# nanoporetech/tombo

Hardware: NVIDIA H100
Metric: resquiggle_reads_per_sec (higher is better)
Workload: dtype f64

## Files before the change

### tombo_b200/csrc/dp_row.cuh

```cuda
#pragma once
#include "common.cuh"

struct DpConsts {
    double z_shift, stay_pen, skip_pen, mhz;
    int winsor;
};

struct RowSpec {
    const double *em;
    const double *zrow;
    double mu, sd;
    tb2_rcp inv_sd;
    int e0;
    int lo, hi;
    double maskval;
};

__device__ __forceinline__ double tb2_zscore(const RowSpec &rs, const DpConsts &c, int j)
{
    if (rs.zrow) return rs.zrow[j];
    if (j < rs.lo || j >= rs.hi) return rs.maskval;
    double a = tb2_div_by(fabs(__ldg(rs.em + (rs.e0 + j)) - rs.mu), rs.sd, rs.inv_sd);
    if (c.winsor) a = (c.mhz < a) ? c.mhz : a;
    return c.z_shift - a;
}

template <int WPL, bool FIX>
__device__ __forceinline__ void tb2_walk(const double *prev, double *cur, int W, int chunk,
                                         int lane, int nvalid, const RowSpec &rs,
                                         const DpConsts &c, int d, bool first_skip, double x,
                                         uint32_t (&codes)[WPL], double &best, int &best_idx,
                                         double &x_end)
{
    const int j0 = lane * chunk;
    int p = j0 + d;
    int lane_p = p / chunk;
    int i_p = p - lane_p * chunk;
    double pm1 = tb2_neg_inf();
    if (p >= 1 && p - 1 < W) {
        const int q = p - 1, lq = q / chunk;
        pm1 = prev[(q - lq * chunk) * 32 + lq];
    }
    bool done = false;
#pragma unroll
    for (int w = 0; w < WPL; ++w) {
        const int ibeg = w * 16;
        const int iend = min(nvalid, ibeg + 16);
        uint32_t cw = FIX ? codes[w] : 0u;
        for (int i = ibeg; i < iend && !done; ++i) {
            const int j = j0 + i;
            const double z = tb2_zscore(rs, c, j);
            const double pv = (p < W) ? prev[i_p * 32 + lane_p] : tb2_neg_inf();
            double nx;
            uint32_t code;
            if (j == 0) {
                if (first_skip) { nx = pv - c.skip_pen; code = 1u; }
                else { nx = pm1 + z; code = 2u; }
            } else {
                const double a = (x - c.stay_pen) + z;
                double cc = pm1 + z;
                uint32_t cf = 2u;
                const double sk = pv - c.skip_pen;
                if (sk > cc) { cc = sk; cf = 1u; }
                if (cc > a) { nx = cc; code = cf; }
                else { nx = a; code = 0u; }
            }
            const int sh = 2 * (i - ibeg);
            if (FIX) {
                const double old = cur[i * 32 + lane];
                cw = (cw & ~(3u << sh)) | (code << sh);
                if (nx == old) done = true;
            } else {
                cw |= code << sh;
            }
            cur[i * 32 + lane] = nx;
            if (nx > best || (FIX && nx == best && j < best_idx)) { best = nx; best_idx = j; }
            x = nx;
            pm1 = pv;
            ++p;
            if (++i_p == chunk) { i_p = 0; ++lane_p; }
        }
        codes[w] = cw;
    }
    if (!done && nvalid > 0) x_end = x;
}

template <int WPL>
__device__ __forceinline__ void tb2_dp_row(const double *prev, double *cur, int W, int chunk,
                                           int lane, const RowSpec &rs, const DpConsts &c,
                                           int d, bool first_skip, uint32_t (&codes)[WPL],
                                           double &best, int &best_idx)
{
    const int nvalid = max(0, min(chunk, W - lane * chunk));
    best = tb2_neg_inf();
    best_idx = 0x7fffffff;
    double x_end = tb2_neg_inf();
    tb2_walk<WPL, false>(prev, cur, W, chunk, lane, nvalid, rs, c, d, first_skip, tb2_neg_inf(),
                         codes, best, best_idx, x_end);
    double last_in = tb2_neg_inf();
    for (;;) {
        const double xin = __shfl_up_sync(TB2_FULL_MASK, x_end, 1);
        const bool need = (lane > 0) && (nvalid > 0) && (xin != last_in);
        if (!__any_sync(TB2_FULL_MASK, need)) break;
        if (need) {
            tb2_walk<WPL, true>(prev, cur, W, chunk, lane, nvalid, rs, c, d, first_skip, xin,
                                codes, best, best_idx, x_end);
            last_in = xin;
        }
    }
}

__device__ __forceinline__ int tb2_warp_argmax(double best, int best_idx)
{
#pragma unroll
    for (int off = 16; off > 0; off >>= 1) {
        const double ob = __shfl_xor_sync(TB2_FULL_MASK, best, off);
        const int oi = __shfl_xor_sync(TB2_FULL_MASK, best_idx, off);
        if (ob > best || (ob == best && oi < best_idx)) { best = ob; best_idx = oi; }
    }
    return best_idx;
}

__device__ unsigned long long g_tb2_dp_counters[8];

#ifdef TB2_EMUL
__device__ __forceinline__ double tb2_lds(unsigned a) { return *(double *)emul_shared_ptr(a); }
__device__ __forceinline__ void tb2_sts(unsigned a, double v) { *(double *)emul_shared_ptr(a) = v; }
#else
__device__ __forceinline__ double tb2_lds(unsigned a)
{
    double v;
    asm volatile("ld.shared.f64 %0, [%1];" : "=d"(v) : "r"(a));
    return v;
}
__device__ __forceinline__ void tb2_sts(unsigned a, double v)
{
    asm volatile("st.shared.f64 [%0], %1;" ::"r"(a), "d"(v));
}
#endif

__device__ __forceinline__ void tb2_dp_row_s(unsigned prev_s, unsigned cur_s, unsigned z_s,
                                             unsigned c_s, int W, int chunk, int lane,
                                             const RowSpec &rs, const DpConsts &c, int d,
                                             bool first_skip, uint32_t &codeword, double &best,
                                             int &best_idx)
{
    const double NEG = tb2_neg_inf();
    const double stay = c.stay_pen, skip = c.skip_pen;
    const int j0 = lane * chunk;
    const int nvalid = max(0, min(chunk, W - j0));
    const unsigned lo8 = 8u * (unsigned)lane;
    cur_s += lo8; z_s += lo8; c_s += lo8;
    uint32_t cfw = 0u, cw = 0u;
    int p = j0 + d;
    int lane_p = p / chunk;
    int i_p = p - lane_p * chunk;
    double pm1 = NEG;
    if (p >= 1 && p - 1 < W) {
        const int q = p - 1, lq = q / chunk;
        pm1 = tb2_lds(prev_s + 8u * (unsigned)((q - lq * chunk) * 32 + lq));
    }
    double x = NEG;
    best = NEG;
    best_idx = 0x7fffffff;
#pragma unroll 1
    for (int i = 0; i < nvalid; ++i) {
        const int j = j0 + i;
        const double zz = tb2_zscore(rs, c, j);
        const double pv = (p < W) ? tb2_lds(prev_s + 8u * (unsigned)(i_p * 32 + lane_p)) : NEG;
        double cand = pm1 + zz;
        uint32_t cf = 2u;
        const double sk = pv - skip;
        double a;
        if (j == 0) {
            a = NEG;
            if (first_skip) { cand = sk; cf = 1u; }
        } else {
            if (sk > cand) { cand = sk; cf = 1u; }
            a = (x - stay) + zz;
        }
        double nx = a;
        uint32_t code = 0u;
        if (cand > a) { nx = cand; code = cf; }
        const unsigned off = 256u * (unsigned)i;
        tb2_sts(z_s + off, zz);
        tb2_sts(c_s + off, cand);
        tb2_sts(cur_s + off, nx);
        cfw |= cf << (2 * i);
        cw |= code << (2 * i);
        if (nx > best) { best = nx; best_idx = j; }
        x = nx;
        pm1 = pv;
        ++p;
        if (++i_p == chunk) { i_p = 0; ++lane_p; }
    }
    double x_end = x;
    double last_in = NEG;
    int n_rounds = 0, n_walked = 0;
    for (;;) {
        const double xin = __shfl_up_sync(TB2_FULL_MASK, x_end, 1);
        const bool need = (lane > 0) && (nvalid > 0) && (xin != last_in);
        if (!__any_sync(TB2_FULL_MASK, need)) break;
        ++n_rounds;
        if (need) {
            double xx = xin;
            bool done = false;
#pragma unroll 1
            for (int i = 0; i < nvalid; ++i) {
                ++n_walked;
                const unsigned off = 256u * (unsigned)i;
                const double a = (xx - stay) + tb2_lds(z_s + off);
                const double cand = tb2_lds(c_s + off);
                double nx = a;
                uint32_t code = 0u;
                if (cand > a) { nx = cand; code = (cfw >> (2 * i)) & 3u; }
                const double old = tb2_lds(cur_s + off);
                cw = (cw & ~(3u << (2 * i))) | (code << (2 * i));
                const int j = j0 + i;
                if (nx > best || (nx == best && j < best_idx)) { best = nx; best_idx = j; }
                xx = nx;
                if (nx == old) { done = true; break; }
                tb2_sts(cur_s + off, nx);
            }
            if (!done) x_end = xx;
            last_in = xin;
        }
    }
    codeword = cw;
#ifdef TB2_DP_COUNTERS
    n_walked = __reduce_add_sync(TB2_FULL_MASK, n_walked);
    if (lane == 0) {
        atomicAdd(&g_tb2_dp_counters[0], 1ULL);
        atomicAdd(&g_tb2_dp_counters[1], (unsigned long long)n_rounds);
        atomicAdd(&g_tb2_dp_counters[2], (unsigned long long)n_walked);
        if (n_rounds > 2) atomicAdd(&g_tb2_dp_counters[3], 1ULL);
    }
#else
    (void)n_rounds; (void)n_walked;
#endif
}

enum { TB2_MODE_PLAIN = 0, TB2_MODE_MASKED = 1, TB2_MODE_ADAPTIVE = 2, TB2_MODE_EXPLICIT = 3 };

struct PassCtx {
    int W, chunk;
    double *buf0, *buf1;
    double *zbuf, *cbuf;
    const double *em;
    int n_em;
    const double *rm, *rs_;
    const double *zmat;
    int mso;
    double msp_start, msp_stop;
    double mask_shifted;
    double mask_fill;
    int *starts;
    uint32_t *tb;
    double *ring;
    double *dbg_fwd;
    long long *dbg_tb;
};

#define TB2_MASK_BASES 50

template <int WPL>
__device__ __noinline__ int tb2_run_rows(const PassCtx &pc, const DpConsts &c, int mode, int r_begin,
                            int r_end, int n_bases_total, int *cur_sel, int *argmax_out)
{
    const int lane = tb2_lane();
    const int W = pc.W, chunk = pc.chunk;
    double *prev = (*cur_sel) ? pc.buf1 : pc.buf0;
    double *cur = (*cur_sel) ? pc.buf0 : pc.buf1;
    int last_argmax = *argmax_out;
    const bool fast_s = (pc.zbuf != nullptr) && __isShared(pc.buf0);
    const unsigned z_s = fast_s ? (unsigned)__cvta_generic_to_shared(pc.zbuf) : 0u;
    const unsigned c_s = fast_s ? (unsigned)__cvta_generic_to_shared(pc.cbuf) : 0u;
    int prev_start = (r_begin > 0) ? pc.starts[r_begin - 1] : 0;
    const int half_bw = W / 2;
    for (int r = r_begin; r < r_end; ++r) {
        RowSpec rs;
        rs.em = pc.em; rs.zrow = nullptr;
        rs.mu = pc.rm ? __ldg(pc.rm + r) : 0.0;
        rs.sd = pc.rs_ ? __ldg(pc.rs_ + r) : 1.0;
        rs.inv_sd = tb2_rcp_of(rs.sd);
        rs.lo = 0; rs.hi = W; rs.maskval = pc.mask_fill;
        int cur_start;
        if (mode == TB2_MODE_ADAPTIVE) {
            cur_start = prev_start + last_argmax - half_bw + 1;
            if (cur_start < prev_start) cur_start = prev_start;
            if (cur_start >= pc.n_em) {
                if (r < n_bases_total - 2) return TB2_ERR_ADAPTIVE_BEYOND_SIGNAL;
                cur_start = pc.n_em - 1;
            }
            if (lane == 0) pc.starts[r] = cur_start;
            rs.hi = min(W, pc.n_em - cur_start);
        } else {
            cur_start = pc.starts[r];
            if (mode == TB2_MODE_MASKED) {
                const int sml = max(pc.mso - cur_start, 0);
                int eml = 0;
                if (r < TB2_MASK_BASES) {
                    const int msp = (int)tb2_linspace_at(pc.msp_start, pc.msp_stop,
                                                         TB2_MASK_BASES, r);
                    eml = W - (msp - cur_start);
                }
                if (cur_start + W - eml > pc.n_em) eml = cur_start + W - pc.n_em;
                rs.lo = sml; rs.hi = W - eml; rs.maskval = pc.mask_shifted;
            } else if (mode == TB2_MODE_EXPLICIT) {
                rs.zrow = pc.zmat + (size_t)r * W;
            }
        }
        rs.e0 = cur_start;
        const int d = (r > 0) ? cur_start - prev_start : 0;
        const bool first_skip = (r == 0) || (d == 0);
        uint32_t codes[WPL];
        double best; int best_idx;
        if (WPL == 1 && fast_s)
            tb2_dp_row_s((unsigned)__cvta_generic_to_shared(prev), (unsigned)__cvta_generic_to_shared(cur),
                         z_s, c_s, W, chunk, lane, rs, c, d, first_skip, codes[0], best, best_idx);
        else
            tb2_dp_row<WPL>(prev, cur, W, chunk, lane, rs, c, d, first_skip, codes, best, best_idx);
#pragma unroll
        for (int w = 0; w < WPL; ++w)
            pc.tb[(size_t)r * (WPL * 32) + w * 32 + lane] = codes[w];
        if (mode == TB2_MODE_ADAPTIVE || r == r_end - 1 || r == n_bases_total - 1)
            last_argmax = tb2_warp_argmax(best, best_idx);
        __syncwarp();
        if (pc.dbg_fwd) {
            const int nvalid = max(0, min(chunk, W - lane * chunk));
            for (int i = 0; i < nvalid; ++i) {
                const int j = lane * chunk + i;
                pc.dbg_fwd[(size_t)(r + 1) * W + j] = cur[i * 32 + lane];
                uint32_t cwv = codes[0];
#pragma unroll
                for (int k = 1; k < WPL; ++k) if ((i >> 4) == k) cwv = codes[k];
                pc.dbg_tb[(size_t)(r + 1) * W + j] = (cwv >> (2 * (i & 15))) & 3u;
            }
        }
        double *t = prev; prev = cur; cur = t;
        *cur_sel ^= 1;
        prev_start = cur_start;
    }
    *argmax_out = last_argmax;
    return TB2_OK;
}

__device__ __forceinline__ void tb2_init_row0(const PassCtx &pc, int *cur_sel)
{
    const int lane = tb2_lane();
    for (int i = 0; i < pc.chunk; ++i) pc.buf0[i * 32 + lane] = 0.0;
    *cur_sel = 0;
    __syncwarp();
}

__device__ __forceinline__ void tb2_load_row(const PassCtx &pc, const double *row, int *cur_sel)
{
    const int lane = tb2_lane();
    for (int j = lane; j < pc.W; j += 32) {
        const int lj = j / pc.chunk;
        pc.buf0[(j - lj * pc.chunk) * 32 + lj] = row[j];
    }
    *cur_sel = 0;
    __syncwarp();
}

template <int WPL>
__device__ __forceinline__ uint32_t tb2_tb_code(const uint32_t (&w)[WPL], int bp, int chunk)
{
    const int lj = bp / chunk;
    const int i = bp - lj * chunk;
    uint32_t v = w[0];
#pragma unroll
    for (int k = 1; k < WPL; ++k) if ((i >> 4) == k) v = w[k];
    v = __shfl_sync(TB2_FULL_MASK, v, lj);
    return (v >> (2 * (i & 15))) & 3u;
}

template <int WPL>
__device__ __noinline__ int tb2_tb_seg_chunk(const uint32_t *tb, const int *starts, int row_hi, int row_lo,
                                int W, int chunk, int thresh, int *cur_event_io, int *read_tb)
{
    const int lane = tb2_lane();
    int cur_event = *cur_event_io;
    int sp = row_hi;
    while (sp > row_lo) {
        const int nblk = min(4, sp - row_lo);
        uint32_t w[4][WPL];
        int st[4];
#pragma unroll
        for (int b = 0; b < 4; ++b) {
            if (b < nblk) {
                const int row = sp - 1 - b;
#pragma unroll
                for (int k = 0; k < WPL; ++k)
                    w[b][k] = tb[(size_t)row * (WPL * 32) + k * 32 + lane];
                st[b] = starts[row];
            }
        }
#pragma unroll
        for (int b = 0; b < 4; ++b) {
            if (b < nblk) {
                int bp = cur_event - st[b];
                if (bp < 0 || bp >= W) return TB2_ERR_UNEXPECTED;
                uint32_t code = tb2_tb_code<WPL>(w[b], bp, chunk);
                while (code == 0u) {
                    --bp;
                    if (bp < 0) return TB2_ERR_UNEXPECTED;
                    code = tb2_tb_code<WPL>(w[b], bp, chunk);
                }
                if (code == 2u) --bp;
                if (thresh >= 0 && min(bp, W - bp - 1) < thresh)
                    return TB2_ERR_BEYOND_BANDWIDTH;
                cur_event = st[b] + bp;
                if (lane == 0) read_tb[sp - 1 - b] = cur_event + 1;
            }
        }
        sp -= nblk;
    }
    *cur_event_io = cur_event;
    __syncwarp();
    return TB2_OK;
}

__device__ __forceinline__ int tb2_wf_strip_words(const int *starts, int s0, int r_end, int W)
{
    const int last = min(31, r_end - 1 - s0);
    const int span = starts[s0 + last] - starts[s0] + W - 1 + last;
    return span < 0 ? -1 : ((span >> 4) + 1) * 32;
}

__device__ long long tb2_wf_total_words(const int *starts, int r_end, int W)
{
    long long sum = 0;
    int bad = 0;
    for (int s0 = tb2_lane() * 32; s0 < r_end; s0 += 32 * 32) {
        const int w = tb2_wf_strip_words(starts, s0, r_end, W);
        if (w < 0) bad = 1; else sum += w;
    }
#pragma unroll
    for (int off = 16; off > 0; off >>= 1) sum += __shfl_xor_sync(TB2_FULL_MASK, sum, off);
    return __any_sync(TB2_FULL_MASK, bad) ? -1 : sum;
}

template <int MODE, bool WIN>
__device__ __forceinline__ double tb2_wf_z(const double *ep, int j, double mu, double sd,
                                           tb2_rcp inv_sd, int lo, int hi, double maskval,
                                           const double *zrow, double zs, double mhz)
{
    if (MODE == TB2_MODE_EXPLICIT) return zrow[j];
    if (MODE == TB2_MODE_MASKED && (j < lo || j >= hi)) return maskval;
    double a = tb2_div_by(fabs(__ldg(ep) - mu), sd, inv_sd);
    if (WIN) a = (mhz < a) ? mhz : a;
    return zs - a;
}

template <bool RBS>
__device__ __forceinline__ double tb2_rb_ld(const double *rb, unsigned rb_s, int i)
{
    if (RBS) return tb2_lds(rb_s + 8u * (unsigned)i);
    return rb[i];
}
template <bool RBS>
__device__ __forceinline__ void tb2_rb_st(double *rb, unsigned rb_s, int i, double v)
{
    if (RBS) tb2_sts(rb_s + 8u * (unsigned)i, v);
    else rb[i] = v;
}

#define TB2_WF_MOVE_BITS(code, q) ((((code) != 0u ? 1u : 0u) << (q)) | (((code) == 1u ? 0x10000u : 0u) << (q)))

#ifdef TB2_EMUL
#define TB2_WF_PLD(up, U) if (l0flag) up = tb2_lds(rd_a + 8 * (U));
#else
#define TB2_WF_PLD(up, U)                                                                       \
        asm volatile("{ .reg .pred p; setp.ne.u32 p, %2, 0; @p ld.shared.f64 %0, [%1+%3]; }"    \
                     : "+d"(up) : "r"(rd_a), "r"(l0flag), "n"(8 * (U)));
#endif
#define TB2_WF_FAST_STEP(U)                                                                     \
    {                                                                                           \
        double up;                                                                              \
        if ((U) == 0) {                                                                         \
            up = __shfl_up_sync(TB2_FULL_MASK, xout, 1);                                        \
            TB2_WF_PLD(up, U)                                                                   \
        } else up = tb2_lds(rd_a + 8u * (U));                                                   \
        __syncwarp();                                                                           \
        const double zn = tb2_wf_z<MODE, WIN>(ep + (U) + 1, j + (U) + 1, mu, sd, inv_sd, lo,    \
                                              hi, maskval, nullptr, zs, mhz);                   \
        const double a = (x - stay) + z;                                                        \
        double cc = up_prev + z;                                                                \
        const double sk = up - skip;                                                            \
        if (sk > cc) { cc = sk; cw |= 0x10000u << (U); }                                        \
        double nx = a;                                                                          \
        if (cc > a) { nx = cc; cw |= 1u << (U); }                                               \
        up_prev = up;                                                                           \
        x = nx; xout = nx; z = zn;                                                              \
        tb2_sts(wr_a + 8u * (U), nx);                                                           \
        __syncwarp();                                                                           \
    }

template <int MODE, bool DBG, bool WIN, bool RBS>
__device__ __noinline__ int tb2_wavefront_rows_t(const PassCtx &pc, const DpConsts &c, int r_end,
                                                 double *rowbuf, uint32_t *tbw, int *argmax_out)
{
    const int lane = tb2_lane();
    const int W = pc.W;
    const double NEG = tb2_neg_inf();
    const double stay = c.stay_pen, skip = c.skip_pen, zs = c.z_shift, mhz = c.mhz;
    const unsigned rb_s = RBS ? (unsigned)__cvta_generic_to_shared(rowbuf) : 0u;
    const unsigned ring_s = (RBS && pc.ring) ? (unsigned)__cvta_generic_to_shared(pc.ring) : 0u;
    const double *em = pc.em;
    const int *starts = pc.starts;
    constexpr bool FAST_T = RBS && !DBG && MODE != TB2_MODE_EXPLICIT;
    const bool FAST = FAST_T && pc.ring != nullptr;
    if (FAST) {
        for (int jj = lane; jj < W; jj += 32) tb2_rb_st<RBS>(rowbuf, rb_s, jj, 0.0);
        __syncwarp();
    }
    uint32_t *tbs = tbw;
    for (int s0 = 0; s0 < r_end; s0 += 32) {
        const int r = s0 + lane;
        const bool row_ok = r < r_end;
        const int lane_last = min(31, r_end - 1 - s0);
        const int rr = min(r, r_end - 1);
        const int start = starts[rr];
        const int prev_start = rr > 0 ? starts[rr - 1] : start;
        const int d = start - prev_start;
        const double mu = pc.rm ? __ldg(pc.rm + rr) : 0.0;
        const double sd = pc.rs_ ? __ldg(pc.rs_ + rr) : 1.0;
        const tb2_rcp inv_sd = tb2_rcp_of(sd);
        int lo = 0, hi = W;
        double maskval = pc.mask_fill;
        if (MODE == TB2_MODE_MASKED && row_ok) {
            const int sml = max(pc.mso - start, 0);
            int eml = 0;
            if (r < TB2_MASK_BASES)
                eml = W - ((int)tb2_linspace_at(pc.msp_start, pc.msp_stop, TB2_MASK_BASES, r) - start);
            if (start + W - eml > pc.n_em) eml = start + W - pc.n_em;
            lo = sml; hi = W - eml; maskval = pc.mask_shifted;
        }
        const double *zrow = (MODE == TB2_MODE_EXPLICIT && row_ok) ? pc.zmat + (size_t)r * W : nullptr;
        const bool first_skip = (r == 0) || (d == 0);
        const bool is_tail = row_ok && (lane == lane_last);
        const int start_first = __shfl_sync(TB2_FULL_MASK, start, 0);
        const int start_last = __shfl_sync(TB2_FULL_MASK, start, lane_last);
        int dmax = row_ok ? d : 0, dmin = row_ok ? d : 0;
#pragma unroll
        for (int off = 16; off > 0; off >>= 1) {
            dmax = max(dmax, __shfl_xor_sync(TB2_FULL_MASK, dmax, off));
            dmin = min(dmin, __shfl_xor_sync(TB2_FULL_MASK, dmin, off));
        }
        const bool lean = FAST && dmin >= 0;
        const int t_begin = start_first;
        const int t_end = start_last + W - 1 + lane_last;
        int t_lo = start_last + lane_last + 1, t_hi = start_first + W - 2 - dmax;
        if (!lean) { t_lo = t_end + 1; t_hi = t_end; }
        double x = 0.0, xout = 0.0, up_prev = 0.0;
        uint32_t cw = 0u;
        const int lane_eff = min(lane, lane_last);
        int j = t_begin - lane_eff - start;
        const double *ep = em + (t_begin - lane_eff);
        int t = t_begin;
        const int w_act = row_ok ? W : 0;
        const int julo = d >= 1 ? 1 : 0, jllo = 1 - julo;
        const unsigned n_u = (unsigned)max(W - d - julo, 0), n_ul = (unsigned)max(W - d - jllo + 1, 0);
#define TB2_WF_LEAN_STEP()                                                                      \
        {                                                                                       \
            double up = __shfl_up_sync(TB2_FULL_MASK, xout, 1);                                 \
            if (lane == 0 && (unsigned)(j + d) < (unsigned)W) up = tb2_rb_ld<RBS>(rowbuf, rb_s, j + d); \
            const double upl = up_prev;                                                         \
            up_prev = up;                                                                       \
            const bool act = (unsigned)j < (unsigned)w_act;                                     \
            const double u = ((unsigned)(j - julo) < n_u) ? up : NEG;                           \
            const double ul = ((unsigned)(j - jllo) < n_ul) ? upl : NEG;                        \
            const double z = act ? tb2_wf_z<MODE, WIN>(ep, j, mu, sd, inv_sd, lo, hi, maskval,  \
                                                       zrow, zs, mhz) : 0.0;                    \
            const double a = (x - stay) + z;                                                    \
            double cc = ul + z;                                                                 \
            uint32_t code = 2u;                                                                 \
            const double sk = u - skip;                                                         \
            if (sk > cc) { cc = sk; code = 1u; }                                                \
            double nx = a;                                                                      \
            if (cc > a) nx = cc; else code = 0u;                                                \
            const int tq = (t - t_begin) & 15;                                                  \
            if (act) {                                                                          \
                x = nx; xout = nx;                                                              \
                cw |= TB2_WF_MOVE_BITS(code, tq);                                               \
                if (is_tail) tb2_rb_st<RBS>(rowbuf, rb_s, j, nx);                               \
            }                                                                                   \
            if (tq == 15 || t == t_end) {                                                       \
                tbs[((t - t_begin) >> 4) * 32 + lane] = cw;                                     \
                cw = 0u;                                                                        \
            }                                                                                   \
              \
              \
            __syncwarp();                                                                       \
            ++j; ++ep;                                                                          \
        }
        if (lean) {
            x = NEG;
            if (lane == 0 && d >= 1) up_prev = tb2_rb_ld<RBS>(rowbuf, rb_s, d - 1);
            for (; t <= t_end && (t < t_lo || ((t - t_begin) & 15) != 0); ++t) TB2_WF_LEAN_STEP()
        }
#define TB2_WF_GENERAL_STEP()                                                                   \
        {                                                                                       \
            double up = __shfl_up_sync(TB2_FULL_MASK, xout, 1);                                 \
            const int p = j + d;                                                                \
            double upl = up_prev;                                                               \
            if (lane == 0) {                                                                    \
                if (s0 == 0) { up = 0.0; upl = 0.0; }                                           \
                else {                                                                          \
                    up = (p >= 0 && p < W) ? tb2_rb_ld<RBS>(rowbuf, rb_s, p) : NEG;             \
                    if (j == 0) upl = (p >= 1 && p - 1 < W) ? tb2_rb_ld<RBS>(rowbuf, rb_s, p - 1) : NEG; \
                }                                                                               \
            }                                                                                   \
            up_prev = up;                                                                       \
            const int tq = (t - t_begin) & 15;                                                  \
            if (row_ok && j >= 0 && j < W) {                                                    \
                const double z = tb2_wf_z<MODE, WIN>(ep, j, mu, sd, inv_sd, lo, hi, maskval,    \
                                                     zrow, zs, mhz);                            \
                const double u = (p < W) ? up : NEG;                                            \
                const double ul = (p >= 1 && p - 1 < W) ? upl : NEG;                            \
                double nx;                                                                      \
                uint32_t code;                                                                  \
                if (j == 0) {                                                                   \
                    if (first_skip) { nx = u - skip; code = 1u; }                               \
                    else { nx = ul + z; code = 2u; }                                            \
                } else {                                                                        \
                    const double a = (x - stay) + z;                                            \
                    double cc = ul + z;                                                         \
                    uint32_t cf = 2u;                                                           \
                    const double sk = u - skip;                                                 \
                    if (sk > cc) { cc = sk; cf = 1u; }                                          \
                    if (cc > a) { nx = cc; code = cf; }                                         \
                    else { nx = a; code = 0u; }                                                 \
                }                                                                               \
                x = nx;                                                                         \
                xout = nx;                                                                      \
                cw |= TB2_WF_MOVE_BITS(code, tq);                                               \
                if (is_tail) tb2_rb_st<RBS>(rowbuf, rb_s, j, nx);                               \
                if (DBG) {                                                                      \
                    pc.dbg_fwd[(size_t)(r + 1) * W + j] = nx;                                   \
                    pc.dbg_tb[(size_t)(r + 1) * W + j] = code;                                  \
                }                                                                               \
            }                                                                                   \
            if (!DBG && (tq == 15 || t == t_end)) {                                             \
                tbs[((t - t_begin) >> 4) * 32 + lane] = cw;                                     \
                cw = 0u;                                                                        \
            }                                                                                   \
            __syncwarp();                                                                       \
            ++j; ++ep;                                                                          \
        }
        if (lean && t + 15 <= t_hi) {
            double z = tb2_wf_z<MODE, WIN>(ep, j, mu, sd, inv_sd, lo, hi, maskval, nullptr, zs, mhz);
            unsigned rd_a = lane == 0 ? rb_s + 8u * (unsigned)(j + d) : ring_s + 8u * (unsigned)(lane - 2);
            unsigned wr_a = is_tail ? rb_s + 8u * (unsigned)j : ring_s + 8u * (unsigned)lane;
            const unsigned rd_inc = lane == 0 ? 128u : 0u, wr_inc = is_tail ? 128u : 0u;
            const unsigned l0flag = lane == 0;
            uint32_t *tbp = tbs + ((t - t_begin) >> 4) * 32 + lane;
            for (; t + 15 <= t_hi; t += 16) {
                TB2_WF_FAST_STEP(0) TB2_WF_FAST_STEP(1) TB2_WF_FAST_STEP(2) TB2_WF_FAST_STEP(3)
                TB2_WF_FAST_STEP(4) TB2_WF_FAST_STEP(5) TB2_WF_FAST_STEP(6) TB2_WF_FAST_STEP(7)
                TB2_WF_FAST_STEP(8) TB2_WF_FAST_STEP(9) TB2_WF_FAST_STEP(10) TB2_WF_FAST_STEP(11)
                TB2_WF_FAST_STEP(12) TB2_WF_FAST_STEP(13) TB2_WF_FAST_STEP(14) TB2_WF_FAST_STEP(15)
                *tbp = cw;
                cw = 0u;
                tbp += 32;
                rd_a += rd_inc; wr_a += wr_inc;
                j += 16; ep += 16;
            }
            cw = 0u;
        }
        if (lean) {
            for (; t <= t_end; ++t) TB2_WF_LEAN_STEP()
        } else {
            for (; t <= t_end; ++t) TB2_WF_GENERAL_STEP()
        }
#undef TB2_WF_GENERAL_STEP
#undef TB2_WF_LEAN_STEP
        tbs += (((t_end - t_begin) >> 4) + 1) * 32;
        __syncwarp();
    }
    double best = NEG;
    int best_idx = 0x7fffffff;
    for (int jj = lane; jj < W; jj += 32) {
        const double v = tb2_rb_ld<RBS>(rowbuf, rb_s, jj);
        if (v > best) { best = v; best_idx = jj; }
    }
    *argmax_out = tb2_warp_argmax(best, best_idx);
    return TB2_OK;
}
#undef TB2_WF_FAST_STEP

__device__ int tb2_wavefront_rows(const PassCtx &pc, const DpConsts &c, int mode, int r_end,
                                  double *rowbuf, uint32_t *tbw, int *argmax_out)
{
    const bool rbs = __isShared(rowbuf);
    const bool win = c.winsor != 0;
#define TB2_WF_CALL(M, D, WN, RB) tb2_wavefront_rows_t<M, D, WN, RB>(pc, c, r_end, rowbuf, tbw, argmax_out)
    if (mode == TB2_MODE_EXPLICIT) {
        if (pc.dbg_fwd) return rbs ? TB2_WF_CALL(TB2_MODE_EXPLICIT, true, false, true)
                                   : TB2_WF_CALL(TB2_MODE_EXPLICIT, true, false, false);
        return TB2_ERR_INVALID_ARG;
    }
    if (mode == TB2_MODE_MASKED) {
        if (win) return rbs ? TB2_WF_CALL(TB2_MODE_MASKED, false, true, true)
                            : TB2_WF_CALL(TB2_MODE_MASKED, false, true, false);
        return rbs ? TB2_WF_CALL(TB2_MODE_MASKED, false, false, true)
                   : TB2_WF_CALL(TB2_MODE_MASKED, false, false, false);
    }
    if (win) return rbs ? TB2_WF_CALL(TB2_MODE_PLAIN, false, true, true)
                        : TB2_WF_CALL(TB2_MODE_PLAIN, false, true, false);
    return rbs ? TB2_WF_CALL(TB2_MODE_PLAIN, false, false, true)
               : TB2_WF_CALL(TB2_MODE_PLAIN, false, false, false);
#undef TB2_WF_CALL
}

__device__ __noinline__ int tb2_tb_seg_wf(const uint32_t *tbw, long long total_words, const int *starts,
                             int n_rows, int W, int thresh, int *cur_event_io, int *read_tb)
{
    const int lane = tb2_lane();
    int cur_event = *cur_event_io;
    const uint32_t *tbs = tbw + total_words;
    for (int s0 = ((n_rows - 1) >> 5) << 5; s0 >= 0; s0 -= 32) {
        const int nblk = min(32, n_rows - s0);
        const int sw = tb2_wf_strip_words(starts, s0, n_rows, W);
        if (sw < 0) return TB2_ERR_UNEXPECTED;
        tbs -= sw;
        const int nw = sw >> 5;
        const int t_begin = starts[s0];
        const float slope = (float)(cur_event - starts[0]) / (float)(s0 + nblk);
        int my_start = 0, base = 0;
        uint32_t w0 = 0, w1 = 0, w2 = 0;
        if (lane < nblk) {
            my_start = starts[s0 + lane];
            const int est = cur_event - (int)((float)(nblk - 1 - lane) * slope) + lane - t_begin;
            base = min(max((est >> 4) - 1, 0), max(nw - 3, 0));
            const uint32_t *rw = tbs + lane;
            w0 = rw[base * 32];
            if (base + 1 < nw) w1 = rw[(base + 1) * 32];
            if (base + 2 < nw) w2 = rw[(base + 2) * 32];
        }
        for (int k = nblk - 1; k >= 0; --k) {
            const int row = s0 + k;
            const int st = __shfl_sync(TB2_FULL_MASK, my_start, k);
            const int bs = __shfl_sync(TB2_FULL_MASK, base, k);
            int bp = cur_event - st;
            if (bp < 0 || bp >= W) return TB2_ERR_UNEXPECTED;
            const int toff = st + k - t_begin;
            uint32_t code;
            for (;;) {
                const int ts = bp + toff;
                const int wi = ts >> 4, rel = wi - bs, q = ts & 15;
                uint32_t v;
                if (rel >= 0 && rel < 3) {
                    const uint32_t mine = rel == 0 ? w0 : (rel == 1 ? w1 : w2);
                    v = __shfl_sync(TB2_FULL_MASK, mine, k);
                } else {
                    v = tbs[wi * 32 + k];
                }
                const uint32_t nz = (v & 0xffffu) & (0xffffu >> (15 - q));
                if (nz != 0u) {
                    const int kq = 31 - __clz(nz);
                    bp -= q - kq;
                    code = ((v >> (16 + kq)) & 1u) ? 1u : 2u;
                    break;
                }
                bp -= q + 1;
                if (bp < 0) return TB2_ERR_UNEXPECTED;
            }
            if (code == 2u) --bp;
            if (thresh >= 0 && min(bp, W - bp - 1) < thresh) return TB2_ERR_BEYOND_BANDWIDTH;
            cur_event = st + bp;
            if (lane == 0) read_tb[row] = cur_event + 1;
        }
    }
    *cur_event_io = cur_event;
    __syncwarp();
    return TB2_OK;
}
```

Measured before the change: 686,500.

## Replace per-step lean edge loop with 16-wide bitmask-predicated edge blocks

The lean wavefront path used to handle its prologue and epilogue diagonals one step at a time, with per-step range checks and a traceback-word store test on every step. These edges now run in 16-step unrolled blocks. Per-block bitmasks (active, load, up, up-left, store) replace the per-step bounds tests, and stores are predicated through inline PTX. The bulk fast loop is kept and interleaved inside the same while loop. This cuts branch and index overhead at the band edges, at the cost of more code size and register pressure plus extra bitmask arithmetic. Optional atomic counters are added behind a compile flag.

```diff
diff --git a/tombo_b200/csrc/dp_row.cuh b/tombo_b200/csrc/dp_row.cuh
--- a/tombo_b200/csrc/dp_row.cuh
+++ b/tombo_b200/csrc/dp_row.cuh
@@ -122,6 +122,12 @@
 }
 
 __device__ unsigned long long g_tb2_dp_counters[8];
+#ifdef TB2_DP_COUNTERS
+__device__ unsigned long long g_tb2_wf_counters[4];
+#define TB2_WF_CNT(i) do { if (tb2_lane() == 0) atomicAdd(&g_tb2_wf_counters[i], 1ULL); } while (0)
+#else
+#define TB2_WF_CNT(i) do { } while (0)
+#endif
 
 #ifdef TB2_EMUL
 __device__ __forceinline__ double tb2_lds(unsigned a) { return *(double *)emul_shared_ptr(a); }
@@ -443,15 +449,30 @@
 }
 
 template <int MODE, bool WIN>
+__device__ __forceinline__ double tb2_wf_z_of(double ev, int j, double mu, double sd,
+                                              tb2_rcp inv_sd, int lo, int hi, double maskval,
+                                              double zs, double mhz)
+{
+    if (MODE == TB2_MODE_MASKED && (j < lo || j >= hi)) return maskval;
+    double a = tb2_div_by(fabs(ev - mu), sd, inv_sd);
+    if (WIN) a = (mhz < a) ? mhz : a;
+    return zs - a;
+}
+template <int MODE, bool WIN>
 __device__ __forceinline__ double tb2_wf_z(const double *ep, int j, double mu, double sd,
                                            tb2_rcp inv_sd, int lo, int hi, double maskval,
                                            const double *zrow, double zs, double mhz)
 {
     if (MODE == TB2_MODE_EXPLICIT) return zrow[j];
     if (MODE == TB2_MODE_MASKED && (j < lo || j >= hi)) return maskval;
-    double a = tb2_div_by(fabs(__ldg(ep) - mu), sd, inv_sd);
-    if (WIN) a = (mhz < a) ? mhz : a;
-    return zs - a;
+    return tb2_wf_z_of<TB2_MODE_PLAIN, WIN>(__ldg(ep), j, mu, sd, inv_sd, lo, hi, maskval, zs, mhz);
+}
+
+__device__ __forceinline__ uint32_t tb2_wf_range_bits(int j0, int lo, int hi)
+{
+    const int a = min(max(lo - j0, 0), 32);
+    const int b = max(min(max(hi - j0, 0), 32), a);
+    return (uint32_t)((1ull << b) - (1ull << a));
 }
 
 template <bool RBS>
@@ -498,6 +519,38 @@
         __syncwarp();                                                                           \
     }
 
+#define TB2_WF_PLDG(v, U) if (m_ld & (2u << (U))) v = __ldg(ep + (U) + 1);
+#ifdef TB2_EMUL
+#define TB2_WF_PST(U, v) if (m_st & (1u << (U))) tb2_sts(wr_a + 8u * (U), v);
+#else
+#define TB2_WF_PST(U, v)                                                                        \
+        asm volatile("{ .reg .pred p; setp.ne.u32 p, %0, 0; @p st.shared.f64 [%1+%2], %3; }"    \
+                     :: "r"(m_st & (1u << (U))), "r"(wr_a), "n"(8 * (U)), "d"(v));
+#endif
+#define TB2_WF_EDGE_STEP(U)                                                                     \
+    {                                                                                           \
+        double up;                                                                              \
+        if ((U) == 0) {                                                                         \
+            up = __shfl_up_sync(TB2_FULL_MASK, xout, 1);                                        \
+            TB2_WF_PLD(up, U)                                                                   \
+        } else up = tb2_lds(rd_a + 8u * (U));                                                   \
+        __syncwarp();                                                                           \
+        TB2_WF_PLDG(ev, U)                                                                      \
+        const double zn = tb2_wf_z_of<MODE, WIN>(ev, j + (U) + 1, mu, sd, inv_sd, lo, hi,       \
+                                                 maskval, zs, mhz);                             \
+        const double ul = (m_ul & (1u << (U))) ? up_prev : NEG;                                 \
+        const double a = (x - stay) + z;                                                        \
+        double cc = ul + z;                                                                     \
+        const double sk = up - skip;                                                            \
+        if ((sk > cc) & ((m_u & (1u << (U))) != 0)) { cc = sk; cw |= 0x10000u << (U); }        \
+        double nx = a;                                                                          \
+        if (cc > a) { nx = cc; cw |= 1u << (U); }                                               \
+        up_prev = up;                                                                           \
+        x = nx; xout = nx; z = zn;                                                              \
+        TB2_WF_PST(U, nx)                                                                       \
+        __syncwarp();                                                                           \
+    }
+
 template <int MODE, bool DBG, bool WIN, bool RBS>
 __device__ __noinline__ int tb2_wavefront_rows_t(const PassCtx &pc, const DpConsts &c, int r_end,
                                                  double *rowbuf, uint32_t *tbw, int *argmax_out)
@@ -552,55 +605,13 @@
         const bool lean = FAST && dmin >= 0;
         const int t_begin = start_first;
         const int t_end = start_last + W - 1 + lane_last;
-        int t_lo = start_last + lane_last + 1, t_hi = start_first + W - 2 - dmax;
-        if (!lean) { t_lo = t_end + 1; t_hi = t_end; }
+        const int t_lo = start_last + lane_last + 1, t_hi = start_first + W - 2 - dmax;
         double x = 0.0, xout = 0.0, up_prev = 0.0;
         uint32_t cw = 0u;
         const int lane_eff = min(lane, lane_last);
         int j = t_begin - lane_eff - start;
         const double *ep = em + (t_begin - lane_eff);
         int t = t_begin;
-        const int w_act = row_ok ? W : 0;
-        const int julo = d >= 1 ? 1 : 0, jllo = 1 - julo;
-        const unsigned n_u = (unsigned)max(W - d - julo, 0), n_ul = (unsigned)max(W - d - jllo + 1, 0);
-#define TB2_WF_LEAN_STEP()                                                                      \
-        {                                                                                       \
-            double up = __shfl_up_sync(TB2_FULL_MASK, xout, 1);                                 \
-            if (lane == 0 && (unsigned)(j + d) < (unsigned)W) up = tb2_rb_ld<RBS>(rowbuf, rb_s, j + d); \
-            const double upl = up_prev;                                                         \
-            up_prev = up;                                                                       \
-            const bool act = (unsigned)j < (unsigned)w_act;                                     \
-            const double u = ((unsigned)(j - julo) < n_u) ? up : NEG;                           \
-            const double ul = ((unsigned)(j - jllo) < n_ul) ? upl : NEG;                        \
-            const double z = act ? tb2_wf_z<MODE, WIN>(ep, j, mu, sd, inv_sd, lo, hi, maskval,  \
-                                                       zrow, zs, mhz) : 0.0;                    \
-            const double a = (x - stay) + z;                                                    \
-            double cc = ul + z;                                                                 \
-            uint32_t code = 2u;                                                                 \
-            const double sk = u - skip;                                                         \
-            if (sk > cc) { cc = sk; code = 1u; }                                                \
-            double nx = a;                                                                      \
-            if (cc > a) nx = cc; else code = 0u;                                                \
-            const int tq = (t - t_begin) & 15;                                                  \
-            if (act) {                                                                          \
-                x = nx; xout = nx;                                                              \
-                cw |= TB2_WF_MOVE_BITS(code, tq);                                               \
-                if (is_tail) tb2_rb_st<RBS>(rowbuf, rb_s, j, nx);                               \
-            }                                                                                   \
-            if (tq == 15 || t == t_end) {                                                       \
-                tbs[((t - t_begin) >> 4) * 32 + lane] = cw;                                     \
-                cw = 0u;                                                                        \
-            }                                                                                   \
-              \
-              \
-            __syncwarp();                                                                       \
-            ++j; ++ep;                                                                          \
-        }
-        if (lean) {
-            x = NEG;
-            if (lane == 0 && d >= 1) up_prev = tb2_rb_ld<RBS>(rowbuf, rb_s, d - 1);
-            for (; t <= t_end && (t < t_lo || ((t - t_begin) & 15) != 0); ++t) TB2_WF_LEAN_STEP()
-        }
 #define TB2_WF_GENERAL_STEP()                                                                   \
         {                                                                                       \
             double up = __shfl_up_sync(TB2_FULL_MASK, xout, 1);                                 \
@@ -650,33 +661,58 @@
             __syncwarp();                                                                       \
             ++j; ++ep;                                                                          \
         }
-        if (lean && t + 15 <= t_hi) {
-            double z = tb2_wf_z<MODE, WIN>(ep, j, mu, sd, inv_sd, lo, hi, maskval, nullptr, zs, mhz);
-            unsigned rd_a = lane == 0 ? rb_s + 8u * (unsigned)(j + d) : ring_s + 8u * (unsigned)(lane - 2);
-            unsigned wr_a = is_tail ? rb_s + 8u * (unsigned)j : ring_s + 8u * (unsigned)lane;
-            const unsigned rd_inc = lane == 0 ? 128u : 0u, wr_inc = is_tail ? 128u : 0u;
+        if (lean) {
+            const int a_hi = row_ok ? W : 0;
+            const int ld_hi = min(hi, a_hi);
+            const int julo = d >= 1 ? 1 : 0, jllo = 1 - julo;
+            x = NEG; xout = NEG;
+            if (lane == 0 && d >= 1) up_prev = tb2_rb_ld<RBS>(rowbuf, rb_s, d - 1);
+            double ev = 0.0;
+            if (tb2_wf_range_bits(j, lo, ld_hi) & 1u) ev = __ldg(ep);
+            double z = tb2_wf_z_of<MODE, WIN>(ev, j, mu, sd, inv_sd, lo, hi, maskval, zs, mhz);
             const unsigned l0flag = lane == 0;
-            uint32_t *tbp = tbs + ((t - t_begin) >> 4) * 32 + lane;
-            for (; t + 15 <= t_hi; t += 16) {
-                TB2_WF_FAST_STEP(0) TB2_WF_FAST_STEP(1) TB2_WF_FAST_STEP(2) TB2_WF_FAST_STEP(3)
-                TB2_WF_FAST_STEP(4) TB2_WF_FAST_STEP(5) TB2_WF_FAST_STEP(6) TB2_WF_FAST_STEP(7)
-                TB2_WF_FAST_STEP(8) TB2_WF_FAST_STEP(9) TB2_WF_FAST_STEP(10) TB2_WF_FAST_STEP(11)
-                TB2_WF_FAST_STEP(12) TB2_WF_FAST_STEP(13) TB2_WF_FAST_STEP(14) TB2_WF_FAST_STEP(15)
-                *tbp = cw;
+            while (t <= t_end) {
+                if (t >= t_lo && t + 15 <= t_hi) {
+                    z = tb2_wf_z<MODE, WIN>(ep, j, mu, sd, inv_sd, lo, hi, maskval, nullptr, zs, mhz);
+                    unsigned rd_a = lane == 0 ? rb_s + 8u * (unsigned)(j + d) : ring_s + 8u * (unsigned)(lane - 2);
+                    unsigned wr_a = is_tail ? rb_s + 8u * (unsigned)j : ring_s + 8u * (unsigned)lane;
+                    const unsigned rd_inc = lane == 0 ? 128u : 0u, wr_inc = is_tail ? 128u : 0u;
+                    uint32_t *tbp = tbs + ((t - t_begin) >> 4) * 32 + lane;
+                    for (; t + 15 <= t_hi; t += 16) {
+                        TB2_WF_FAST_STEP(0) TB2_WF_FAST_STEP(1) TB2_WF_FAST_STEP(2) TB2_WF_FAST_STEP(3)
+                        TB2_WF_FAST_STEP(4) TB2_WF_FAST_STEP(5) TB2_WF_FAST_STEP(6) TB2_WF_FAST_STEP(7)
+                        TB2_WF_FAST_STEP(8) TB2_WF_FAST_STEP(9) TB2_WF_FAST_STEP(10) TB2_WF_FAST_STEP(11)
+                        TB2_WF_FAST_STEP(12) TB2_WF_FAST_STEP(13) TB2_WF_FAST_STEP(14) TB2_WF_FAST_STEP(15)
+                        *tbp = cw;
+                        cw = 0u;
+                        tbp += 32;
+                        rd_a += rd_inc; wr_a += wr_inc;
+                        j += 16; ep += 16;
+                        TB2_WF_CNT(MODE == TB2_MODE_MASKED ? 3 : 1);
+                    }
+                    continue;
+                }
+                const uint32_t m_act = tb2_wf_range_bits(j, 0, a_hi);
+                const uint32_t m_ld = tb2_wf_range_bits(j, lo, ld_hi);
+                const uint32_t m_u = tb2_wf_range_bits(j, julo, W - d);
+                const uint32_t m_ul = tb2_wf_range_bits(j, jllo, W - d + 1);
+                const uint32_t m_st = is_tail ? m_act : 0xffffffffu;
+                const unsigned rd_a = lane == 0 ? rb_s + 8u * (unsigned)min(j + d, W)
+                                                : ring_s + 8u * (unsigned)(lane - 2);
+                const unsigned wr_a = is_tail ? rb_s + 8u * (unsigned)j : ring_s + 8u * (unsigned)lane;
+                TB2_WF_EDGE_STEP(0) TB2_WF_EDGE_STEP(1) TB2_WF_EDGE_STEP(2) TB2_WF_EDGE_STEP(3)
+                TB2_WF_EDGE_STEP(4) TB2_WF_EDGE_STEP(5) TB2_WF_EDGE_STEP(6) TB2_WF_EDGE_STEP(7)
+                TB2_WF_EDGE_STEP(8) TB2_WF_EDGE_STEP(9) TB2_WF_EDGE_STEP(10) TB2_WF_EDGE_STEP(11)
+                TB2_WF_EDGE_STEP(12) TB2_WF_EDGE_STEP(13) TB2_WF_EDGE_STEP(14) TB2_WF_EDGE_STEP(15)
+                tbs[((t - t_begin) >> 4) * 32 + lane] = cw & ((m_act & 0xffffu) * 0x10001u);
                 cw = 0u;
-                tbp += 32;
-                rd_a += rd_inc; wr_a += wr_inc;
-                j += 16; ep += 16;
-            }
-            cw = 0u;
-        }
-        if (lean) {
-            for (; t <= t_end; ++t) TB2_WF_LEAN_STEP()
+                t += 16; j += 16; ep += 16;
+                TB2_WF_CNT(MODE == TB2_MODE_MASKED ? 2 : 0);
+            }
         } else {
             for (; t <= t_end; ++t) TB2_WF_GENERAL_STEP()
         }
 #undef TB2_WF_GENERAL_STEP
-#undef TB2_WF_LEAN_STEP
         tbs += (((t_end - t_begin) >> 4) + 1) * 32;
         __syncwarp();
     }
@@ -690,6 +726,9 @@
     return TB2_OK;
 }
 #undef TB2_WF_FAST_STEP
+#undef TB2_WF_EDGE_STEP
+#undef TB2_WF_PLDG
+#undef TB2_WF_PST
 
 __device__ int tb2_wavefront_rows(const PassCtx &pc, const DpConsts &c, int mode, int r_end,
                                   double *rowbuf, uint32_t *tbw, int *argmax_out)
```

New measurement: 725,200 (median of 6 runs). 5.6% higher.
